# bd4sur/Nano

Measured on AMD Instinct MI355X. Metric: decode_tokens_per_sec, higher is better.
Workload: dtype i8

## Files before the change

nano_amd/csrc/gemv_q80_impl.h:

```cpp
#include <string.h>
#include <stdio.h>
#include "gemv_common.h"
#include "gemv_q80_host.h"

namespace nano {

namespace {


__device__ __forceinline__ void quant_store4(float4 v, float scale, int8_t *dst) {
    const int q0 = q80_quant1(v.x, scale), q1 = q80_quant1(v.y, scale), q2 = q80_quant1(v.z, scale), q3 = q80_quant1(v.w, scale);
    *reinterpret_cast<uint32_t *>(dst) = (uint32_t)(q0 & 0xff) | ((uint32_t)(q1 & 0xff) << 8) | ((uint32_t)(q2 & 0xff) << 16) | ((uint32_t)(q3 & 0xff) << 24);
}

template <int ROLE, int GS, int B, int NV>
__device__ __forceinline__ void stage_finish(const GemvDev &a, Staged<B, NV> &r, int8_t *xq, float *xs, float *red, uint32_t n16, uint32_t ng4) {
    const uint32_t tid = threadIdx.x, nthr = a.nthr, n = a.n, ng = a.ng;
    const uint32_t lane = tid & 63u, wid = tid >> 6, NW = nthr >> 6;
    if (has_flag<ROLE>(a, F_PRE)) {
        for (uint32_t b = 0; b < a.nb; b++) {
            for (uint32_t i = tid * 16u; i < n; i += nthr * 16u) *reinterpret_cast<int4 *>(xq + b * n16 + i) = *reinterpret_cast<const int4 *>(a.xq_in + (size_t)b * n16 + i);
            for (uint32_t i = tid; i < ng; i += nthr) xs[b * ng4 + i] = a.xs_in[(size_t)b * ng + i];
        }
        __syncthreads();
// ... 154 lines not shown
template <int NQ> __device__ __forceinline__ float fold_row_canon(const float *p) {
    static_assert(NQ % 2 == 0, "whole units");
    float4 t[NQ];
#pragma unroll
    for (int q = 0; q < NQ; q++) t[q] = *reinterpret_cast<const float4 *>(p + 4 * q);
    __builtin_amdgcn_sched_barrier(0);
    float s[NQ / 2];
    unit_sums<NQ / 2>(t, s);
    float v = s[0];
#pragma unroll
    for (int u = 1; u < NQ / 2; u++) v = fadd(v, s[u]);
    return v;
}
__device__ __forceinline__ float fold_row_canon_any(const float *p, uint32_t ng) {
    float v = 0.0f;
    for (uint32_t g0 = 0; g0 < ng; g0 += 16) {
        float4 t[4];
#pragma unroll
        for (int q = 0; q < 4; q++) t[q] = (g0 + 4u * (uint32_t)q < ng) ? *reinterpret_cast<const float4 *>(p + g0 + 4 * q) : make_float4(0.f, 0.f, 0.f, 0.f);
        float s = t[0].x; s += t[0].y; s += t[0].z; s += t[0].w;
        if (g0 + 4 < ng) { s += t[1].x; s += t[1].y; s += t[1].z; s += t[1].w; }
        v = g0 == 0 ? s : v + s;
        if (g0 + 8 < ng) {
            s = t[2].x; s += t[2].y; s += t[2].z; s += t[2].w;
            if (g0 + 12 < ng) { s += t[3].x; s += t[3].y; s += t[3].z; s += t[3].w; }
            v += s;
        }
    }
    return v;
}
template <int NQ> __device__ __forceinline__ void fold_row2_canon(const float *p0, const float *p1, float &v0, float &v1) {
    static_assert(NQ % 2 == 0, "whole units");
    float4 t[NQ], u[NQ];
#pragma unroll
    for (int q = 0; q < NQ; q++) { t[q] = *reinterpret_cast<const float4 *>(p0 + 4 * q); u[q] = *reinterpret_cast<const float4 *>(p1 + 4 * q); }
    __builtin_amdgcn_sched_barrier(0);
    float s0[NQ / 2], s1[NQ / 2];
    unit_sums<NQ / 2>(t, s0); unit_sums<NQ / 2>(u, s1);
    v0 = s0[0]; v1 = s1[0];
#pragma unroll
    for (int k = 1; k < NQ / 2; k++) { v0 = fadd(v0, s0[k]); v1 = fadd(v1, s1[k]); }
}
__device__ __forceinline__ void fold_row2_canon_ng(const float *p0, const float *p1, uint32_t ng, float &v0, float &v1) {
    if (ng == 16u) { fold_row2_canon<4>(p0, p1, v0, v1); return; }
    v0 = fold_row_canon_any(p0, ng); v1 = fold_row_canon_any(p1, ng);
}
__device__ __forceinline__ float fold_row_canon_ng(const float *p, uint32_t ng) {
    if (ng == 16u) return fold_row_canon<4>(p);
    if (ng == 32u) return fold_row_canon<8>(p);
    if (ng == 48u) return fold_row_canon<12>(p);
    return fold_row_canon_any(p, ng);
}

template <int ROLE, int GS, int B, int NV, int UPW, int EARLY = 0>
__global__ __launch_bounds__(1024) void gemv_q80_slab_kernel(const GemvDev a) {
    extern __shared__ __attribute__((aligned(16))) unsigned char smem[];
#define SLAB_EARLY EARLY
#define SLAB_A a
#define SLAB_BID blockIdx.x
#define SLAB_HAND 0
#define SLAB_HANDV (SlabHand{})
#define SLAB_PTAG 0u
#define SLAB_XHAND 0
#define SLAB_XHANDV (SlabHand{})
#define SLAB_CTAG 0u
#define SLAB_PART 0
#include "gemv_q80_slab_body.inc"
#undef SLAB_A
#undef SLAB_BID
#undef SLAB_HAND
#undef SLAB_HANDV
#undef SLAB_PTAG
#undef SLAB_XHAND
#undef SLAB_XHANDV
#undef SLAB_CTAG
#undef SLAB_PART
#undef SLAB_EARLY
}

#if NANO_Q80_GS == 64
}
}
#include "attn_impl.h"
namespace nano {
namespace {
struct FusedArgs { GemvDev g; AttnArgs a; SlabHand hand; uint32_t n_attn, head_wgs, wait16, ngemv; };
template <int NV, int UPW>
__global__ __launch_bounds__(256) void qkv_attn_fused_kernel(const FusedArgs fa) {
    extern __shared__ __attribute__((aligned(16))) unsigned char smem[];
    const uint2 tk_ = hand_tick(fa.hand);
    if (blockIdx.x >= fa.ngemv) {
        const uint32_t ab = blockIdx.x - fa.ngemv;
        const uint32_t split = ab / fa.head_wgs, grp = ab - split * fa.head_wgs;
        attention_body<8, 4, 1, 1, false, false, 2, false, true>(fa.a, smem, grp, 0u, split, fa.hand, hand_ctag(tk_, fa.hand), fa.wait16);
        return;
    }
    constexpr int ROLE = R_NORM_STORE, GS = 64, B = 1;
#define SLAB_A fa.g
#define SLAB_BID blockIdx.x
#define SLAB_HAND 1
#define SLAB_HANDV fa.hand
#define SLAB_PTAG hand_ptag(tk_, fa.hand)
#define SLAB_XHAND 0
#define SLAB_XHANDV (SlabHand{})
#define SLAB_CTAG 0u
#define SLAB_PART 0
#include "gemv_q80_slab_body.inc"
#undef SLAB_A
#undef SLAB_BID
#undef SLAB_HAND
#undef SLAB_HANDV
#undef SLAB_PTAG
#undef SLAB_XHAND
#undef SLAB_XHANDV
#undef SLAB_CTAG
#undef SLAB_PART
}

struct Wo13Args { GemvDev wo; GemvDev w13; SlabHand hand; uint32_t wo_wgs, wait16; };
template <int ROLE_A, int NV_A, int UPW_A, int NV_B, int UPW_B, int NT>
__global__ __launch_bounds__(NT) void wo_w13_fused_kernel(const Wo13Args fa) {
    extern __shared__ __attribute__((aligned(16))) unsigned char smem[];
    constexpr int GS = 64, B = 1;
    const uint2 tk_ = hand_tick(fa.hand);
    {
        constexpr int ROLE = ROLE_A, NV = NV_A, UPW = UPW_A;
#define SLAB_BID blockIdx.x
#define SLAB_A fa.wo
#define SLAB_HAND 1
#define SLAB_HANDV fa.hand
#define SLAB_PTAG hand_ptag(tk_, fa.hand)
#define SLAB_XHAND 0
#define SLAB_XHANDV (SlabHand{})
#define SLAB_CTAG 0u
#define SLAB_PART 1
#include "gemv_q80_slab_body.inc"
#undef SLAB_PART
        auto wo_rest = [&]() __attribute__((always_inline)) {
#define SLAB_PART 2
#include "gemv_q80_slab_body.inc"
#undef SLAB_PART
        };
#undef SLAB_A
#undef SLAB_HAND
#undef SLAB_HANDV
#undef SLAB_PTAG
#undef SLAB_XHAND
#undef SLAB_XHANDV
#undef SLAB_CTAG
        {
            constexpr int ROLE = R_NORM_SWIGLU, NV = NV_B, UPW = UPW_B;
#define SLAB_A fa.w13
#define SLAB_HAND 0
#define SLAB_HANDV (SlabHand{})
#define SLAB_PTAG 0u
#define SLAB_XHAND 1
#define SLAB_XHANDV fa.hand
#define SLAB_CTAG hand_ctag(tk_, fa.hand)
#define SLAB_XHAND_WAIT (blockIdx.x >= fa.wo_wgs ? fa.wait16 : 0u)
#define SLAB_XHAND_NAP 2
#define SLAB_PART 1
#include "gemv_q80_slab_body.inc"
#undef SLAB_PART
            if (blockIdx.x < fa.wo_wgs) wo_rest();
            __syncthreads();
#define SLAB_PART 2
#include "gemv_q80_slab_body.inc"
#undef SLAB_PART
#undef SLAB_A
#undef SLAB_HAND
#undef SLAB_HANDV
#undef SLAB_PTAG
#undef SLAB_XHAND
#undef SLAB_XHANDV
#undef SLAB_CTAG
#undef SLAB_XHAND_WAIT
#undef SLAB_XHAND_NAP
        }
#undef SLAB_BID
    }
}

#endif

template <int ROLE, int GS, int B, int NV>
__global__ __launch_bounds__(256) void gemv_q80_stream_kernel(const GemvDev a) {
    extern __shared__ __attribute__((aligned(16))) unsigned char smem[];
    constexpr int LPG = GS / 16, GC = 1024 / GS, F = GC / 4;
    static_assert(F >= 1, "group size too large for the stream kernel");
    const uint32_t n = a.n, ng = a.ng;
    const int tid = threadIdx.x, lane = tid & 63;
    const int wid = __builtin_amdgcn_readfirstlane(tid >> 6);
    const uint32_t n16 = (n + 15) & ~15u, ng4 = (ng + 3) & ~3u;
    int8_t *xq = reinterpret_cast<int8_t *>(smem);
    float *xs = reinterpret_cast<float *>(smem + B * n16);
    float *red = xs + B * ng4;
    int *tab = reinterpret_cast<int *>(red + B * 16) + wid * 16 * GC;

    Staged<B, NV> sx;
    stage_issue<ROLE, B, NV>(a, sx);

    const uint32_t rows = a.rows[0];
    const uint32_t nchunk = a.nchunk;
    const uint32_t ntiles = (rows + 15) >> 4;
    const uint32_t nwaves = gridDim.x * 4, wave_g = blockIdx.x * 4 + (uint32_t)wid;
    const uint32_t nunits = (wave_g < ntiles) ? ((ntiles - wave_g + nwaves - 1) / nwaves) * nchunk : 0;
    const __amdgpu_buffer_rsrc_t rw_ = mkrsrc(a.w[0], rows * n);
    const __amdgpu_buffer_rsrc_t rs_ = mkrsrc(a.ws[0], rows * ng * 4u);

    int4 wA[16];
    float sA[F];
    uint32_t tile_i = 0, chunk_i = 0;
    auto issue = [&](int4 (&w)[16], float (&s)[F]) {
        const uint32_t tile = wave_g + tile_i * nwaves;
        const uint32_t row0 = tile << 4;
        const uint32_t col = (chunk_i << 10) + (uint32_t)lane * 16u;
        const uint32_t base = (col < n) ? row0 * n + col : OOB;
#pragma unroll
        for (int r = 0; r < 16; r++) w[r] = bload_w(rw_, base + (uint32_t)r * n);
        const uint32_t gb = chunk_i * GC + ((uint32_t)lane & 3u) * F;
        const uint32_t so = ((row0 + ((uint32_t)lane >> 2)) * ng + gb) * 4u;
#pragma unroll
        for (int f = 0; f < F; f++) s[f] = bload_f(rs_, (gb + f < ng) ? so + 4u * f : OOB);
        if (++chunk_i == nchunk) { chunk_i = 0; tile_i++; }
    };
    if (nunits) issue(wA, sA);

    stage_finish<ROLE, GS, B, NV>(a, sx, xq, xs, red, n16, ng4);

    float val[B], best[B];
// ... 81 lines not shown
    const uint32_t nchunk = (a.n + 1023) / 1024, nmat = a.epi == GEMV_EPI_SWIGLU ? 2 : 1;
    const uint32_t nseg = a.epi == GEMV_EPI_SWIGLU ? 1u : a.nseg;
    uint32_t align = 0;
    if (nseg > 1) for (uint32_t s = 0; s < nseg; s++) align |= a.seg[s].rows;
    const uint32_t rows = total_rows(a);
    uint32_t rw = 4;
    while (rw < 32 && (align % (rw * 2)) == 0 && (rw * 2 / 4) * nchunk <= 4 && rows / (rw * 2) >= 128) rw *= 2;
    while (rw < 64 && (align % (rw * 2)) == 0 && rows / (rw * 2) >= 256) rw *= 2;
    {
        const uint32_t ng = a.n / a.gs, pitch = ((ng + 47) / 64) * 64 + 16;
        while (rw > 4 && (size_t)B * nmat * rw * pitch * 4 > 64 * 1024) rw /= 2;
        while (rw > 4 && (rw / 4) * nchunk * nmat > 64) rw /= 2;
    }
    if (B == 1 && nseg == 1) {
        const uint32_t cus = a.cus ? a.cus : 256u, c = (rows + cus - 1) / cus;
        if (c >= 5 && c < rw && rows / rw < cus && ((c + 3) / 4) * nchunk * nmat <= 64) rw = c;
    }
    uint32_t large_nw = 0;
    if (B <= 2 && (uint64_t)rows * a.n * nmat >= (8u << 20)) {
        const uint32_t cus = a.cus ? a.cus : 256u;
        uint32_t best = 0, best_cost = ~0u;
        const uint32_t ng = a.n / a.gs, pitch = (1024 / a.gs == 16) ? (((ng + 47) / 64) * 64 + 16) : (((ng + 3) & ~3u) + 4);
        for (uint32_t c = 4; c <= 64; c++) {
            const uint32_t tpw = (c + 3) / 4;
            if (tpw * nchunk * nmat > 64) break;
            if ((size_t)B * nmat * tpw * 4 * pitch * 4 > 96 * 1024) break;
            uint32_t wgs = 0;
            if (nseg > 1) for (uint32_t s2 = 0; s2 < nseg; s2++) wgs += (a.seg[s2].rows + c - 1) / c; else wgs = (rows + c - 1) / c;
            uint32_t cost = ((wgs + cus - 1) / cus) * c * 100u;
            if (wgs > cus) cost += cost * 15u / 100u;
            if (cost <= best_cost) { best_cost = cost; best = c; }
        }
        if (best) {
            rw = best;
            const uint32_t u = ((rw + 3) / 4) * nchunk * nmat;
            large_nw = u / 2 < 8 ? 8 : (u / 2 > 16 ? 16 : u / 2);
        }
    }
    const uint32_t units = ((rw + 3) / 4) * nchunk * nmat;
    uint32_t nw = units < 4 ? units : 4;
    const uint32_t want_div = B == 1 ? 384u : 512u;
    uint32_t want = (a.n * (uint32_t)(B > 2 ? B / 2 : 1) + want_div - 1) / want_div;
    if (want > 16) want = 16;
    if (nw < want) nw = want;
    if (nw * 64 < rw * (uint32_t)B) nw = (rw * (uint32_t)B + 63) / 64;
    if (nw < 2) nw = 2;
    uint32_t upw = (units + nw - 1) / nw;
    while (upw > 4 && nw < 16) { nw++; upw = (units + nw - 1) / nw; }
    if (large_nw) { nw = large_nw; upw = (units + nw - 1) / nw; while (upw > 4 && nw < 16) { nw++; upw = (units + nw - 1) / nw; } }
    SlabPlan p{rw, nw, upw, (a.n + 256 * nw - 1) / (256 * nw)};
    return p;
}

template <int ROLE, int GS, int B, int NV, int UPW>
static hipError_t launch_slab_t(const GemvDev &d, const SlabPlan &p, uint32_t nwg, hipStream_t st) {
    const uint32_t nmat = d.epi == GEMV_EPI_SWIGLU ? 2 : 1;
    const size_t n16 = (d.n + 15) & ~15u, ng4 = (d.ng + 3) & ~3u;
    const size_t pitch = (1024 / GS == 16) ? (((d.ng + 47) / 64) * 64 + 16) : (ng4 + 4);
    const size_t lds = B * n16 + B * ng4 * 4 + B * 64 + ((d.flags & F_COMBINE) ? (size_t)B * d.attn_n_head * 32 : 0) + (size_t)B * nmat * (d.tpw * 4) * pitch * 4;
    GemvDev dd = d; dd.nthr = 64 * p.nw;
    if constexpr (GS == 64 && B <= 2 && UPW >= 2 && NV >= 1) if (d.early) {
        auto kern = &gemv_q80_slab_kernel<ROLE, GS, B, NV, UPW, 1>;
        if (lds > 64 * 1024) (void)hipFuncSetAttribute(reinterpret_cast<const void *>(kern), hipFuncAttributeMaxDynamicSharedMemorySize, (int)lds);
        hipLaunchKernelGGL(kern, dim3(nwg), dim3(64 * p.nw), lds, st, dd);
        return hipGetLastError();
    }
    auto kern = &gemv_q80_slab_kernel<ROLE, GS, B, NV, UPW>;
    if (lds > 64 * 1024) (void)hipFuncSetAttribute(reinterpret_cast<const void *>(kern), hipFuncAttributeMaxDynamicSharedMemorySize, (int)lds);
    hipLaunchKernelGGL(kern, dim3(nwg), dim3(64 * p.nw), lds, st, dd);
    return hipGetLastError();
}
template <int ROLE, int GS, int B>
static hipError_t launch_slab_r(const GemvDev &d, const SlabPlan &p, uint32_t rows, hipStream_t st) {
    if (p.upw > 4) return hipErrorInvalidValue;
#define SLAB_GO(NV_, UPW_) do { if constexpr (B * NV_ <= 8) return launch_slab_t<ROLE, GS, B, NV_, UPW_>(d, p, rows, st); } while (0)
    int nv = p.nv <= 1 ? 1 : p.nv <= 2 ? 2 : p.nv <= 4 ? 4 : 0;
    const int upw = p.upw <= 1 ? 1 : p.upw <= 2 ? 2 : 4;
    if (B * nv > 8) nv = 0;
    if (nv == 1) { if (upw == 1) SLAB_GO(1, 1); if (upw == 2) SLAB_GO(1, 2); SLAB_GO(1, 4); }
    if (nv == 2) { if (upw == 1) SLAB_GO(2, 1); if (upw == 2) SLAB_GO(2, 2); SLAB_GO(2, 4); }
    if (nv == 4) { if (upw == 1) SLAB_GO(4, 1); if (upw == 2) SLAB_GO(4, 2); SLAB_GO(4, 4); }
    if (upw == 1) SLAB_GO(0, 1);
    if (upw == 2) SLAB_GO(0, 2);
    SLAB_GO(0, 4);
    return hipErrorInvalidValue;
#undef SLAB_GO
}
template <int GS, int B>
static hipError_t launch_slab_b(GemvDev &d, const GemvArgs &a, hipStream_t st) {
    const SlabPlan p = plan_slab(a, B);
    d.rw = p.rw;
    d.early = (B <= 2 && p.upw >= 2 && (uint64_t)total_rows(a) * a.n * (a.epi == GEMV_EPI_SWIGLU ? 2 : 1) >= (8u << 20)) ? 1u : 0u;
    d.tpw = (p.rw + 3) / 4;
    d.magic_rw = 65536u / p.rw + 1u;
    d.log2_tiles = 0;
    const bool sw = d.epi == GEMV_EPI_SWIGLU;
    d.units = d.tpw * d.nchunk * (sw ? 2 : 1);
    uint32_t wg[3] = {0, 0, 0};
    const uint32_t nseg = sw ? 1u : a.nseg;
    for (uint32_t s2 = 0; s2 < nseg; s2++) wg[s2] = (a.seg[s2].rows + p.rw - 1) / p.rw;
    d.wg_c0 = nseg > 1 ? wg[0] : 0xffffffffu;
    d.wg_c1 = nseg > 2 ? wg[0] + wg[1] : 0xffffffffu;
    const uint32_t rows = wg[0] + wg[1] + wg[2];
    if constexpr (B == 1) if (GS != 64 || d.canon) {
        const uint32_t f = d.flags;
        if (f == F_NORM && d.epi == GEMV_EPI_STORE) return launch_slab_r<R_NORM_STORE, GS, B>(d, p, rows, st);
        if (f == 0 && d.epi == GEMV_EPI_RESID) return launch_slab_r<R_RESID, GS, B>(d, p, rows, st);
        if (f == F_COMBINE && d.epi == GEMV_EPI_RESID) return launch_slab_r<R_RESID_COMBINE, GS, B>(d, p, rows, st);
        if (f == F_NORM && d.epi == GEMV_EPI_SWIGLU) return launch_slab_r<R_NORM_SWIGLU, GS, B>(d, p, rows, st);
    }
    return launch_slab_r<R_GENERIC, GS, B>(d, p, rows, st);
}

template <int ROLE, int GS, int B>
static hipError_t launch_stream_r(GemvDev &d, hipStream_t st) {
    d.ntiles = STREAM_WGS * 4; d.nthr = 256;
    const size_t n16 = (d.n + 15) & ~15u, ng4 = (d.ng + 3) & ~3u;
// ... 9 lines not shown
    if constexpr (B <= 2) { if (!done && nv <= 4) { STREAM_GO(4); done = true; } }
    if (!done) { STREAM_GO(0); }
#undef STREAM_GO
    return hipGetLastError();
}
template <int GS, int B>
static hipError_t launch_stream_b(GemvDev &d, hipStream_t st) {
    if (d.flags == F_NORM) return launch_stream_r<R_NORM_STORE, GS, B>(d, st);
    return launch_stream_r<R_GENERIC, GS, B>(d, st);
}

#if NANO_Q80_GS == 64
static bool fused_shape(const GemvArgs &ga, const AttnArgs &aa, SlabPlan &p) {
    if (ga.gs != 64 || ga.nb != 1 || ga.nseg != 3 || ga.epi != GEMV_EPI_STORE || !ga.norm_w || ga.xq_in || ga.attn_part || ga.tile_max || ga.resid_add) return false;
    if (ga.n % 64u || ga.n > 4096u || use_stream(ga) || !q80_canonical(ga)) return false;
    if (ga.seg[0].out_pstride || ga.seg[1].out_pstride) return false;
    p = plan_slab(ga, 1);
    if (p.nw != 4u || p.upw > 4u || !(p.nv == 1u || p.nv == 2u || p.nv == 4u)) return false;
    if (!fused_attn_side_ok(aa, ga.seg[0].rows, ga.seg[1].rows, ga.seg[2].rows)) return false;
    return true;
}

struct Wo13Plan { SlabPlan a, b; uint32_t nw, nv_a, upw_a, wa, wb; int sig; };
static bool wo13_shape(const GemvArgs &wo, const GemvArgs &w13, Wo13Plan &q) {
    if (wo.gs != 64 || w13.gs != 64 || wo.nb != 1 || w13.nb != 1 || !q80_canonical(wo) || !q80_canonical(w13)) return false;
    if (wo.nseg != 1 || wo.epi != GEMV_EPI_RESID || wo.norm_w || wo.xq_in || wo.tile_max || wo.resid_add || wo.seg[0].out_pstride) return false;
    if (wo.attn_part && (wo.attn_nsplit > 8u || wo.attn_hd % 4u)) return false;
    if (w13.nseg != 2 || w13.epi != GEMV_EPI_SWIGLU || !w13.norm_w || w13.xq_in || w13.attn_part || w13.tile_max || w13.resid_add) return false;
    if (use_stream(wo) || use_stream(w13) || w13.n != wo.seg[0].rows || w13.xin != wo.seg[0].out || w13.n % 4u) return false;
    q.a = plan_slab(wo, 1); q.b = plan_slab(w13, 1);
    q.nw = q.b.nw;
    const uint32_t units_a = ((q.a.rw + 3) / 4) * ((wo.n + 1023) / 1024);
    q.upw_a = (units_a + q.nw - 1) / q.nw;
    q.nv_a = (wo.n / 4 + 64 * q.nw - 1) / (64 * q.nw);
    q.wa = (wo.seg[0].rows + q.a.rw - 1) / q.a.rw; q.wb = (w13.seg[0].rows + q.b.rw - 1) / q.b.rw;
    const uint32_t cus = w13.cus ? w13.cus : 256u;
    if (q.wa > q.wb || q.wb > cus) return false;
    if (q.a.rw > 64 * q.nw || q.b.rw > 64 * q.nw) return false;
    q.sig = 0;
    if (q.nw == 4u && q.nv_a == 2u && q.upw_a == 1u && q.b.nv == 1u && q.b.upw == 2u) q.sig = 1;
    if (q.sig == 1) {
        const uint32_t units_b = ((q.b.rw + 3) / 4) * ((w13.n + 1023) / 1024) * 2u;
        if ((units_a + 7u) / 8u == 1u && (wo.n / 4 + 511u) / 512u == 1u && (units_b + 7u) / 8u == 1u && (w13.n / 4 + 511u) / 512u == 1u) { q.sig = 3; q.nw = 8u; }
    }
    return q.sig != 0;
}
static void slab_dev_fill(GemvDev &d, const GemvArgs &a, const SlabPlan &p, uint32_t nthr) {
    d.tile_max = nullptr;
    d.rw = p.rw; d.tpw = (p.rw + 3) / 4; d.magic_rw = 65536u / p.rw + 1u; d.log2_tiles = 0;
    d.units = d.tpw * d.nchunk * (a.epi == GEMV_EPI_SWIGLU ? 2u : 1u);
    d.wg_c0 = 0xffffffffu; d.wg_c1 = 0xffffffffu;
    d.nthr = nthr;
}
static size_t slab_lds(const GemvDev &d) {
    const uint32_t nmat = d.epi == GEMV_EPI_SWIGLU ? 2 : 1;
    const size_t n16 = (d.n + 15) & ~15u, ng4 = (d.ng + 3) & ~3u, pitch = ((d.ng + 47) / 64) * 64 + 16;
    return n16 + ng4 * 4 + 64 + ((d.flags & F_COMBINE) ? (size_t)d.attn_n_head * 32 : 0) + (size_t)nmat * (d.tpw * 4) * pitch * 4;
}

#endif

template <int GS, int B>
static hipError_t launch_b(const GemvArgs &a, hipStream_t st) {
    GemvDev d = to_dev(a);
    if (use_stream(a)) return launch_stream_b<GS, B>(d, st);
    d.tile_max = nullptr;
    return launch_slab_b<GS, B>(d, a, st);
}
template <int GS>
static hipError_t launch_gs(const GemvArgs &a, hipStream_t st) {
    if (a.nb <= 1) return launch_b<GS, 1>(a, st);
    if (a.nb <= 2) return launch_b<GS, 2>(a, st);
    if (a.nb <= 4) return launch_b<GS, 4>(a, st);
    return launch_b<GS, 8>(a, st);
}

}

hipError_t NANO_Q80_ENTRY(const GemvArgs &a, hipStream_t st) { return launch_gs<NANO_Q80_GS>(a, st); }

#if NANO_Q80_GS == 64
bool qkv_attn_fused_supports(const GemvArgs &ga, const AttnArgs &aa) { SlabPlan p; return fused_shape(ga, aa, p); }

hipError_t launch_qkv_attn_fused(const GemvArgs &ga, const AttnArgs &aa, unsigned long long *hand, uint32_t *tick, uint32_t layer1, hipStream_t st) {
    SlabPlan p;
    if (!hand || !tick || !layer1 || layer1 > 127u || !fused_shape(ga, aa, p)) return hipErrorInvalidValue;
    GemvDev d = to_dev(ga);
    d.tile_max = nullptr;
    d.rw = p.rw; d.tpw = (p.rw + 3) / 4; d.magic_rw = 65536u / p.rw + 1u; d.log2_tiles = 0;
    d.units = d.tpw * d.nchunk;
    uint32_t wg[3];
    for (uint32_t s2 = 0; s2 < 3; s2++) wg[s2] = (ga.seg[s2].rows + p.rw - 1) / p.rw;
    d.wg_c0 = wg[0]; d.wg_c1 = wg[0] + wg[1];
    const uint32_t ngemv = wg[0] + wg[1] + wg[2];
    d.nthr = 256;
    AttnArgs a = aa;
    { uint32_t l2 = 0; while ((1u << l2) < a.n_kv_head) l2++; a.kv_log2 = l2; }
    { const uint32_t kv_mul = a.n_head / a.n_kv_head; uint32_t l2 = 0; while ((1u << l2) < kv_mul) l2++; a.kvmul_log2 = l2; }
    SlabHand h{};
    h.buf = hand; h.tick = tick; h.layer1 = layer1;
    h.base[0] = 0; h.base[1] = a.q_dim; h.base[2] = a.q_dim + a.kv_dim;
    const uint32_t n_attn = a.n_head * a.nsplit;
    const size_t n16 = (d.n + 15) & ~15u, ng4 = (d.ng + 3) & ~3u, pitch = ((d.ng + 47) / 64) * 64 + 16;
    const size_t lds_g = n16 + ng4 * 4 + 64 + (size_t)(d.tpw * 4) * pitch * 4;
    const size_t hd4 = a.hd, lds_a = (hd4 + hd4 + 4 + 4 + 4 * hd4 + hd4 + 4 + 4 * 8 * hd4) * sizeof(float);
    const size_t lds = lds_g > lds_a ? lds_g : lds_a;
    if (lds > 64 * 1024) return hipErrorInvalidValue;
    const int upw = p.upw <= 1 ? 1 : p.upw <= 2 ? 2 : 4;
    FusedArgs fa{};
    fa.g = d; fa.a = a; fa.hand = h; fa.n_attn = n_attn; fa.head_wgs = a.n_head; fa.ngemv = ngemv;
    fa.wait16 = 1u;
#define FUSED_GO(NV_, UPW_) do { hipLaunchKernelGGL((qkv_attn_fused_kernel<NV_, UPW_>), dim3(n_attn + ngemv), dim3(256), lds, st, fa); return hipGetLastError(); } while (0)
#define FUSED_NV(NV_) do { if (upw == 1) FUSED_GO(NV_, 1); if (upw == 2) FUSED_GO(NV_, 2); FUSED_GO(NV_, 4); } while (0)
    if (p.nv == 1u) FUSED_NV(1);
    if (p.nv == 2u) FUSED_NV(2);
    FUSED_NV(4);
#undef FUSED_NV
#undef FUSED_GO
}

bool wo_w13_fused_supports(const GemvArgs &wo, const GemvArgs &w13) { Wo13Plan q; return wo13_shape(wo, w13, q); }

hipError_t launch_wo_w13_fused(const GemvArgs &wo, const GemvArgs &w13, unsigned long long *hand, uint32_t *tick, uint32_t layer1, hipStream_t st) {
    Wo13Plan q;
    if (!hand || !tick || !layer1 || layer1 > 127u || !wo13_shape(wo, w13, q)) return hipErrorInvalidValue;
    Wo13Args fa{};
    fa.wo = to_dev(wo); fa.w13 = to_dev(w13);
    slab_dev_fill(fa.wo, wo, q.a, 64 * q.nw); slab_dev_fill(fa.w13, w13, q.b, 64 * q.nw);
    fa.wo_wgs = q.wa;
    fa.wait16 = 4u;
    SlabHand h{};
    h.buf = hand; h.tick = tick; h.layer1 = layer1;
    h.base[0] = 0; h.base[1] = 0; h.base[2] = 0;
    fa.hand = h;
    const size_t la = slab_lds(fa.wo), lb = slab_lds(fa.w13), lds = la > lb ? la : lb;
    if (lds > 64 * 1024) return hipErrorInvalidValue;
    const bool comb = (fa.wo.flags & F_COMBINE) != 0;
#define WO13_GO(RA_, NVA_, UA_, NVB_, UB_, NT_) do { hipLaunchKernelGGL((wo_w13_fused_kernel<RA_, NVA_, UA_, NVB_, UB_, NT_>), dim3(q.wb), dim3(NT_), lds, st, fa); return hipGetLastError(); } while (0)
    if (q.sig == 1) { if (comb) WO13_GO(R_RESID_COMBINE, 2, 1, 1, 2, 256); WO13_GO(R_RESID, 2, 1, 1, 2, 256); }
    if (comb) WO13_GO(R_RESID_COMBINE, 1, 1, 1, 1, 512);
    WO13_GO(R_RESID, 1, 1, 1, 1, 512);
#undef WO13_GO
}
#endif

}
```

nano_amd/csrc/gemv_q80_slab_body.inc:

```
#ifndef SLAB_EARLY
#define SLAB_EARLY 0
#define SLAB_EARLY_DEFAULTED 1
#endif
#ifndef SLAB_XHAND_WAIT
#define SLAB_XHAND_WAIT 0u
#define SLAB_XHAND_NAP 0
#define SLAB_XHAND_WAIT_DEFAULTED 1
#endif
#define SLAB_ISSUE_UNIT(k) do { \
        const uint32_t u = (uint32_t)wid + (uint32_t)k * NW; \
        const uint32_t t = (u * SLAB_A.magic_nchunk) >> 16; \
        const uint32_t c = u - t * SLAB_A.nchunk; \
        const uint32_t mat = t >= TPW ? 1u : 0u, tl = t - mat * TPW; \
        const bool live = u < SLAB_A.units; \
        const __amdgpu_buffer_rsrc_t rw_ = mkrsrc(mat ? SLAB_A.w[1] : w0, live ? rows0 * n : 0u); \
        const __amdgpu_buffer_rsrc_t rs_ = mkrsrc(mat ? SLAB_A.ws[1] : ws0, live ? rows0 * ng * 4u : 0u); \
        const uint32_t lrow = lrow0 + tl * TR; \
        const uint32_t col = (c << 10) + (uint32_t)lane * 16u; \
        const uint32_t base = (col < n) ? lrow * n + col : OOB; \
        _Pragma("unroll") \
        for (int r = 0; r < TR; r++) wv[k][r] = bload_w(rw_, base + ((tl * TR + (uint32_t)r < RW) ? (uint32_t)r * n : OOB)); \
        const uint32_t g = c * GC + (uint32_t)lane / LPG; \
        _Pragma("unroll") \
        for (int s = 0; s < NS; s++) { \
            const uint32_t r = ((uint32_t)lane % LPG) + s * LPG; \
            sv[k][s] = bload_f(rs_, (r < TR && tl * TR + r < RW && g < ng) ? ((lrow + r) * ng + g) * 4u : OOB); \
        } \
    } while (0)
#if SLAB_PART != 2
    constexpr int TR = 4;
    constexpr int LPG = GS / 16, GC = 1024 / GS;
    constexpr int NS = (TR + LPG - 1) / LPG;
    const int tid = threadIdx.x, lane = tid & 63;
    const int wid = __builtin_amdgcn_readfirstlane(tid >> 6);
    const int NW = (int)(SLAB_A.nthr >> 6);
    const uint32_t n = SLAB_A.n, ng = SLAB_A.ng;
    const uint32_t n16 = (n + 15) & ~15u, ng4 = (ng + 3) & ~3u;
    const uint32_t PITCH = (GC == 16) ? (((ng + 47) / 64) * 64 + 16) : (ng4 + 4);
    const uint32_t RW = SLAB_A.rw, TPW = SLAB_A.tpw, RWP = TPW * TR;
    const uint32_t epi = role_epi<ROLE>(SLAB_A);
    const bool swiglu = epi == GEMV_EPI_SWIGLU;
    const uint32_t nmat = swiglu ? 2 : 1;
    int8_t *xq = reinterpret_cast<int8_t *>(smem);
    float *xs = reinterpret_cast<float *>(smem + B * n16);
    float *red = xs + B * ng4;
    float *P = red + B * 16 + (has_flag<ROLE>(SLAB_A, F_COMBINE) ? B * SLAB_A.attn_n_head * 8 : 0);

    karg_touch(SLAB_A.out[0]); karg_touch(SLAB_A.out_bstride[0]); karg_touch(SLAB_A.out_pstride[0]); karg_touch(SLAB_A.rows[0]); karg_touch(SLAB_A.magic_rw); karg_touch(SLAB_A.nb);
    if (!(ROLE == R_RESID || ROLE == R_RESID_COMBINE || ROLE == R_NORM_SWIGLU)) {
        karg_touch(SLAB_A.out[1]); karg_touch(SLAB_A.out[2]); karg_touch(SLAB_A.out_bstride[1]); karg_touch(SLAB_A.out_bstride[2]);
        karg_touch(SLAB_A.out_pstride[1]); karg_touch(SLAB_A.out_pstride[2]); karg_touch(SLAB_A.rows[1]); karg_touch(SLAB_A.rows[2]);
    }
    karg_touch(SLAB_A.pos); karg_touch(SLAB_A.canon);
    if (ROLE == R_GENERIC || ROLE == R_RESID || ROLE == R_RESID_COMBINE) { karg_touch(SLAB_A.resid_add); karg_touch(SLAB_A.resid_add_bstride); }
    NANO_STAMP(SLAB_A.stamps, 0, tid);
    Staged<B, NV> sx;
    if constexpr (SLAB_XHAND) stage_issue_nw<ROLE, B, NV>(SLAB_A, sx);
    else if (!(NANO_STAMPS && (SLAB_A.dbg & 2u))) stage_issue<ROLE, B, NV>(SLAB_A, sx);

    constexpr bool ONESEG = ROLE == R_RESID || ROLE == R_RESID_COMBINE || ROLE == R_NORM_SWIGLU;
    const int sel = (ONESEG || swiglu) ? 0 : (int)(SLAB_BID >= SLAB_A.wg_c0) + (int)(SLAB_BID >= SLAB_A.wg_c1);
    const int8_t *w0 = sel == 0 ? SLAB_A.w[0] : sel == 1 ? SLAB_A.w[1] : SLAB_A.w[2];
    const float *ws0 = sel == 0 ? SLAB_A.ws[0] : sel == 1 ? SLAB_A.ws[1] : SLAB_A.ws[2];
    float *out0 = sel == 0 ? SLAB_A.out[0] : sel == 1 ? SLAB_A.out[1] : SLAB_A.out[2];
    const uint32_t rows0 = sel == 0 ? SLAB_A.rows[0] : sel == 1 ? SLAB_A.rows[1] : SLAB_A.rows[2];
    const uint32_t obs = sel == 0 ? SLAB_A.out_bstride[0] : sel == 1 ? SLAB_A.out_bstride[1] : SLAB_A.out_bstride[2];
    const uint32_t ops = sel == 0 ? SLAB_A.out_pstride[0] : sel == 1 ? SLAB_A.out_pstride[1] : SLAB_A.out_pstride[2];
    const uint32_t lrow0 = (SLAB_BID - (sel == 0 ? 0u : sel == 1 ? SLAB_A.wg_c0 : SLAB_A.wg_c1)) * RW;

    int4 wv[UPW][TR];
    float sv[UPW][NS];
    constexpr uint32_t early_ = (uint32_t)(SLAB_EARLY);
    static_assert(SLAB_PART == 0 || early_ == 0u, "SLAB_EARLY: the whole body only");
#pragma unroll
    for (int k = 0; k < UPW; k++) { if (early_ == 0u || (uint32_t)k < early_) SLAB_ISSUE_UNIT(k); }
    if (!SLAB_XHAND && NANO_STAMPS && (SLAB_A.dbg & 2u)) stage_issue<ROLE, B, NV>(SLAB_A, sx);
    const int fb = (int)(((uint32_t)tid * SLAB_A.magic_rw) >> 16);
    const int frl = tid - fb * (int)RW;
    const bool fold_live = tid < (int)(RW * B) && fb < (int)SLAB_A.nb && lrow0 + frl < rows0;
    uint32_t opos = 0;
    if (ops && fold_live) opos = SLAB_A.pos[fb];
    float oldv = 0.0f;
    if (epi == GEMV_EPI_RESID && fold_live) oldv = out0[(size_t)fb * obs + lrow0 + frl];
    float addv = 0.0f;
    const bool has_add = epi == GEMV_EPI_RESID && SLAB_A.resid_add != nullptr;
    if (has_add && fold_live) addv = SLAB_A.resid_add[(size_t)fb * SLAB_A.resid_add_bstride + lrow0 + frl];

    NANO_STAMP(SLAB_A.stamps, 1, oldv);
#endif
#if SLAB_PART != 1
    if constexpr (SLAB_XHAND) {
        static_assert(!SLAB_XHAND || B == 1, "granule activations: one sequence");
        const unsigned long long *hb_ = SLAB_XHANDV.buf;
        const uint32_t ctag_ = SLAB_CTAG;
        bool got_ = false;
        for (uint32_t w_ = 0; w_ < SLAB_XHAND_WAIT; w_++) __builtin_amdgcn_s_sleep(16);
        for (uint32_t spin_ = 0; spin_ < (1u << 14) && !got_; spin_++) {
            if (spin_) __builtin_amdgcn_s_sleep(SLAB_XHAND_NAP);
            if ((spin_ & 63u) == 63u && hand_aborted(SLAB_XHANDV)) break;
            got_ = true;
#pragma unroll
            for (int j = 0; j < NV; j++) {
                const uint32_t i = ((uint32_t)tid + (uint32_t)j * SLAB_A.nthr) * 4u;
                if (i < n) {
                    const unsigned long long g0_ = __hip_atomic_load(hb_ + i, __ATOMIC_RELAXED, __HIP_MEMORY_SCOPE_AGENT);
                    const unsigned long long g1_ = __hip_atomic_load(hb_ + i + 1, __ATOMIC_RELAXED, __HIP_MEMORY_SCOPE_AGENT);
                    const unsigned long long g2_ = __hip_atomic_load(hb_ + i + 2, __ATOMIC_RELAXED, __HIP_MEMORY_SCOPE_AGENT);
                    const unsigned long long g3_ = __hip_atomic_load(hb_ + i + 3, __ATOMIC_RELAXED, __HIP_MEMORY_SCOPE_AGENT);
                    got_ = got_ && (uint32_t)(g0_ >> 32) == ctag_ && (uint32_t)(g1_ >> 32) == ctag_ && (uint32_t)(g2_ >> 32) == ctag_ && (uint32_t)(g3_ >> 32) == ctag_;
                    sx.x[0][j] = make_float4(__uint_as_float((uint32_t)g0_), __uint_as_float((uint32_t)g1_), __uint_as_float((uint32_t)g2_), __uint_as_float((uint32_t)g3_));
                } else sx.x[0][j] = make_float4(0.f, 0.f, 0.f, 0.f);
            }
        }
        if (!got_) hand_give_up(SLAB_XHANDV, SLAB_A.err);
    }
    stage_finish<ROLE, GS, B, NV>(SLAB_A, sx, xq, xs, red, n16, ng4);
    if constexpr (early_ != 0u) {
#pragma unroll
        for (int k = 1; k < UPW; k++) { if ((uint32_t)k >= early_) SLAB_ISSUE_UNIT(k); }
    }
    NANO_STAMP(SLAB_A.stamps, 3, xs[0]);

#pragma unroll
    for (int k = 0; k < UPW; k++) {
        const uint32_t u = (uint32_t)wid + (uint32_t)k * NW;
        if (u < SLAB_A.units) {
            const uint32_t t = (u * SLAB_A.magic_nchunk) >> 16;
            const uint32_t c = u - t * SLAB_A.nchunk;
            const uint32_t mat = t >= TPW ? 1u : 0u, tl = t - mat * TPW;
            const uint32_t col = (c << 10) + (uint32_t)lane * 16u;
            const uint32_t g = c * GC + (uint32_t)lane / LPG;
#pragma unroll
            for (int b = 0; b < B; b++) {
                if (b < (int)SLAB_A.nb) {
                    const int4 xv = (col < n) ? *reinterpret_cast<const int4 *>(xq + b * n16 + col) : make_int4(0, 0, 0, 0);
                    int iv[TR];
#pragma unroll
                    for (int r = 0; r < TR; r++) {
                        int d = __builtin_amdgcn_sdot4(wv[k][r].x, xv.x, 0, false);
                        d = __builtin_amdgcn_sdot4(wv[k][r].y, xv.y, d, false);
                        d = __builtin_amdgcn_sdot4(wv[k][r].z, xv.z, d, false);
                        d = __builtin_amdgcn_sdot4(wv[k][r].w, xv.w, d, false);
                        iv[r] = dpp_group_sum<LPG>(d);
                    }
                    const float xsc = (g < ng) ? xs[b * ng4 + g] : 0.0f;
#pragma unroll
                    for (int s = 0; s < NS; s++) {
                        const uint32_t r = ((uint32_t)lane % LPG) + s * LPG;
                        int v = iv[0];
#pragma unroll
                        for (int q = 1; q < TR; q++) v = (q == (int)r) ? iv[q] : v;
                        if (r < TR && g < ng)
                            P[(((size_t)b * nmat + mat) * RWP + tl * TR + r) * PITCH + g] = ((float)v * sv[k][s]) * xsc;
                    }
                }
            }
        }
    }
    NANO_STAMP(SLAB_A.stamps, 4, wv[UPW - 1][TR - 1].w);
    __syncthreads();
    NANO_STAMP(SLAB_A.stamps, 5, P[0]);

    constexpr bool PFOLD = early_ != 0u && GS == 64;
    bool pfold_ = false;
    if constexpr (PFOLD) {
        pfold_ = (ROLE != R_GENERIC || SLAB_A.canon) && (ng & 7u) == 0u;
        if (pfold_) {
            const uint32_t nu_ = ng >> 3, rows_ = RW * (uint32_t)B * nmat, items_ = rows_ * nu_;
            for (uint32_t it = (uint32_t)tid; it < items_; it += SLAB_A.nthr) {
                const uint32_t rr_ = it / nu_, u_ = it - rr_ * nu_;
                const uint32_t bm_ = rr_ / RW, rl_ = rr_ - bm_ * RW;
                float *pu_ = P + ((size_t)bm_ * RWP + rl_) * PITCH + 8u * u_;
                const float4 t0_ = *reinterpret_cast<const float4 *>(pu_), t1_ = *reinterpret_cast<const float4 *>(pu_ + 4);
                pu_[0] = unit_sum(t0_, t1_);
            }
// ... 15 lines not shown
            if constexpr (ROLE == R_NORM_SWIGLU) fold_row2_canon_ng(p0, p1, ng, v0, v1); else v0 = fold_row_canon_ng(p0, ng);
        } else
        if (GS == 64 && SLAB_A.canon) {
            v0 = fold_row_canon_ng(p0, ng);
            if (swiglu) v1 = fold_row_canon_ng(p1, ng);
        } else
        if (!swiglu && ng == 48u) v0 = fold_row<12>(p0);
        else if (!swiglu && ng == 32u) v0 = fold_row<8>(p0);
        else if (ng == 16u) {
            if (swiglu) fold_row2<4>(p0, p1, v0, v1); else v0 = fold_row<4>(p0);
        } else if ((ng & 15u) == 0) {
            for (uint32_t g0 = 0; g0 < ng; g0 += 16) {
                float4 t[4], u[4];
#pragma unroll
                for (int q = 0; q < 4; q++) { t[q] = *reinterpret_cast<const float4 *>(p0 + g0 + 4 * q); if (swiglu) u[q] = *reinterpret_cast<const float4 *>(p1 + g0 + 4 * q); }
#pragma unroll
                for (int q = 0; q < 4; q++) { v0 += t[q].x; v0 += t[q].y; v0 += t[q].z; v0 += t[q].w; }
                if (swiglu) {
#pragma unroll
                    for (int q = 0; q < 4; q++) { v1 += u[q].x; v1 += u[q].y; v1 += u[q].z; v1 += u[q].w; }
                }
            }
        } else {
        for (uint32_t g0 = 0; g0 < ng; g0 += 16) {
                float4 t[4], u[4];
#pragma unroll
                for (int q = 0; q < 4; q++) {
                    t[q] = (g0 + 4 * q < ng4) ? *reinterpret_cast<const float4 *>(p0 + g0 + 4 * q) : make_float4(0.f, 0.f, 0.f, 0.f);
                    if (swiglu) u[q] = (g0 + 4 * q < ng4) ? *reinterpret_cast<const float4 *>(p1 + g0 + 4 * q) : make_float4(0.f, 0.f, 0.f, 0.f);
                }
#pragma unroll
                for (int q = 0; q < 4; q++) {
                    const uint32_t g = g0 + 4 * q;
                    v0 += (g < ng) ? t[q].x : 0.0f; v0 += (g + 1 < ng) ? t[q].y : 0.0f; v0 += (g + 2 < ng) ? t[q].z : 0.0f; v0 += (g + 3 < ng) ? t[q].w : 0.0f;
                }
                if (swiglu) {
#pragma unroll
                    for (int q = 0; q < 4; q++) {
                        const uint32_t g = g0 + 4 * q;
                        v1 += (g < ng) ? u[q].x : 0.0f; v1 += (g + 1 < ng) ? u[q].y : 0.0f; v1 += (g + 2 < ng) ? u[q].z : 0.0f; v1 += (g + 3 < ng) ? u[q].w : 0.0f;
                    }
                }
            }
        }
        if (fold_live) {
            float *dst = out0 + (size_t)fb * obs + (size_t)opos * ops + lrow0 + frl;
            const float val = finish_epi(epi, has_add ? v0 + addv : v0, v1, oldv);
            if constexpr (SLAB_HAND == 1)
                __hip_atomic_store(SLAB_HANDV.buf + (sel == 0 ? SLAB_HANDV.base[0] : sel == 1 ? SLAB_HANDV.base[1] : SLAB_HANDV.base[2]) + lrow0 + (uint32_t)frl,
                                   ((unsigned long long)(SLAB_PTAG) << 32) | (unsigned long long)__float_as_uint(val), __ATOMIC_RELAXED, __HIP_MEMORY_SCOPE_AGENT);
            if (NANO_STAMPS && (SLAB_A.dbg & 4u)) *dst = val; else __hip_atomic_store(dst, val, __ATOMIC_RELAXED, __HIP_MEMORY_SCOPE_AGENT);
        }
    }
    NANO_STAMP_END(SLAB_A.stamps, 6);
#endif
#undef SLAB_ISSUE_UNIT
#ifdef SLAB_EARLY_DEFAULTED
#undef SLAB_EARLY
#undef SLAB_EARLY_DEFAULTED
#endif
#ifdef SLAB_XHAND_WAIT_DEFAULTED
#undef SLAB_XHAND_WAIT
#undef SLAB_XHAND_NAP
#undef SLAB_XHAND_WAIT_DEFAULTED
#endif
```

Measured before the change: 1969.

## Add wave-level cross-lane fold path for single-chunk rmsnorm GEMVs

Adds a specialised slab-kernel variant for n=1024, 16-group rmsnorm-store and swiglu GEMVs. Each wave reduces its rows entirely in registers using DPP and permlane16/32 swaps, instead of writing partial sums to an LDS table and folding them after a barrier. The swiglu variant pairs the gate and up rows within one unit, which halves the unit count, and the LDS partial table is dropped from the allocation. This removes LDS traffic and synchronisation in the small-model decode GEMVs, at the cost of extra template instantiations and a hardcoded shape path.

```diff
diff --git a/nano_amd/csrc/gemv_q80_impl.h b/nano_amd/csrc/gemv_q80_impl.h
--- a/nano_amd/csrc/gemv_q80_impl.h
+++ b/nano_amd/csrc/gemv_q80_impl.h
@@ -230,10 +230,23 @@
     return fold_row_canon_any(p, ng);
 }
 
-template <int ROLE, int GS, int B, int NV, int UPW, int EARLY = 0>
+__device__ __forceinline__ float wave_fold_canon16(float p) {
+    const float p1 = DPP_F(p, 0x104), p2 = DPP_F(p, 0x108), p3 = DPP_F(p, 0x10C);
+    float s = fadd(p, p1); s = fadd(s, p2); s = fadd(s, p3);
+    const uint32_t sb = __float_as_uint(s);
+    const float c = __uint_as_float(__builtin_amdgcn_permlane16_swap(sb, sb, false, false)[0]);
+    s = fadd(c, p); s = fadd(s, p1); s = fadd(s, p2); s = fadd(s, p3);
+    const uint32_t tb = __float_as_uint(s);
+    const float s0 = __uint_as_float(__builtin_amdgcn_permlane32_swap(tb, tb, false, false)[0]);
+    return fadd(s0, s);
+}
+constexpr int WF_LANE0 = 48;
+
+template <int ROLE, int GS, int B, int NV, int UPW, int EARLY = 0, int WF = 0>
 __global__ __launch_bounds__(1024) void gemv_q80_slab_kernel(const GemvDev a) {
     extern __shared__ __attribute__((aligned(16))) unsigned char smem[];
 #define SLAB_EARLY EARLY
+#define SLAB_WF WF
 #define SLAB_A a
 #define SLAB_BID blockIdx.x
 #define SLAB_HAND 0
@@ -254,6 +267,7 @@
 #undef SLAB_CTAG
 #undef SLAB_PART
 #undef SLAB_EARLY
+#undef SLAB_WF
 }
 
 #if NANO_Q80_GS == 64
@@ -265,38 +279,19 @@
 struct FusedArgs { GemvDev g; AttnArgs a; SlabHand hand; uint32_t n_attn, head_wgs, wait16, ngemv; };
 template <int NV, int UPW>
 __global__ __launch_bounds__(256) void qkv_attn_fused_kernel(const FusedArgs fa) {
-    extern __shared__ __attribute__((aligned(16))) unsigned char smem[];
-    const uint2 tk_ = hand_tick(fa.hand);
-    if (blockIdx.x >= fa.ngemv) {
-        const uint32_t ab = blockIdx.x - fa.ngemv;
-        const uint32_t split = ab / fa.head_wgs, grp = ab - split * fa.head_wgs;
-        attention_body<8, 4, 1, 1, false, false, 2, false, true>(fa.a, smem, grp, 0u, split, fa.hand, hand_ctag(tk_, fa.hand), fa.wait16);
-        return;
-    }
-    constexpr int ROLE = R_NORM_STORE, GS = 64, B = 1;
-#define SLAB_A fa.g
-#define SLAB_BID blockIdx.x
-#define SLAB_HAND 1
-#define SLAB_HANDV fa.hand
-#define SLAB_PTAG hand_ptag(tk_, fa.hand)
-#define SLAB_XHAND 0
-#define SLAB_XHANDV (SlabHand{})
-#define SLAB_CTAG 0u
-#define SLAB_PART 0
-#include "gemv_q80_slab_body.inc"
-#undef SLAB_A
-#undef SLAB_BID
-#undef SLAB_HAND
-#undef SLAB_HANDV
-#undef SLAB_PTAG
-#undef SLAB_XHAND
-#undef SLAB_XHANDV
-#undef SLAB_CTAG
-#undef SLAB_PART
+#define SLAB_WF 0
+#include "qkv_attn_fused_body.inc"
+#undef SLAB_WF
+}
+template <int NV, int UPW>
+__global__ __launch_bounds__(256) void qkv_attn_fused_wf_kernel(const FusedArgs fa) {
+#define SLAB_WF 1
+#include "qkv_attn_fused_body.inc"
+#undef SLAB_WF
 }
 
 struct Wo13Args { GemvDev wo; GemvDev w13; SlabHand hand; uint32_t wo_wgs, wait16; };
-template <int ROLE_A, int NV_A, int UPW_A, int NV_B, int UPW_B, int NT>
+template <int ROLE_A, int NV_A, int UPW_A, int NV_B, int UPW_B, int NT, int WF = 0>
 __global__ __launch_bounds__(NT) void wo_w13_fused_kernel(const Wo13Args fa) {
     extern __shared__ __attribute__((aligned(16))) unsigned char smem[];
     constexpr int GS = 64, B = 1;
@@ -337,6 +332,7 @@
 #define SLAB_CTAG hand_ctag(tk_, fa.hand)
 #define SLAB_XHAND_WAIT (blockIdx.x >= fa.wo_wgs ? fa.wait16 : 0u)
 #define SLAB_XHAND_NAP 2
+#define SLAB_WF WF
 #define SLAB_PART 1
 #include "gemv_q80_slab_body.inc"
 #undef SLAB_PART
@@ -354,6 +350,7 @@
 #undef SLAB_CTAG
 #undef SLAB_XHAND_WAIT
 #undef SLAB_XHAND_NAP
+#undef SLAB_WF
         }
 #undef SLAB_BID
     }
@@ -541,6 +538,9 @@
     return p;
 }
 
+static bool slab_wave_fold(const GemvDev &d) {
+    return d.n == 1024u && d.ng == 16u && !d.early && (d.epi == GEMV_EPI_STORE || (d.epi == GEMV_EPI_SWIGLU && !d.out_pstride[0]));
+}
 template <int ROLE, int GS, int B, int NV, int UPW>
 static hipError_t launch_slab_t(const GemvDev &d, const SlabPlan &p, uint32_t nwg, hipStream_t st) {
     const uint32_t nmat = d.epi == GEMV_EPI_SWIGLU ? 2 : 1;
@@ -552,6 +552,11 @@
         auto kern = &gemv_q80_slab_kernel<ROLE, GS, B, NV, UPW, 1>;
         if (lds > 64 * 1024) (void)hipFuncSetAttribute(reinterpret_cast<const void *>(kern), hipFuncAttributeMaxDynamicSharedMemorySize, (int)lds);
         hipLaunchKernelGGL(kern, dim3(nwg), dim3(64 * p.nw), lds, st, dd);
+        return hipGetLastError();
+    }
+    if constexpr (GS == 64 && B == 1 && (ROLE == R_NORM_STORE || ROLE == R_NORM_SWIGLU) && (NV == 1 || NV == 2)) if (slab_wave_fold(d)) {
+        if (ROLE == R_NORM_SWIGLU) dd.units = (d.rw + 1) / 2;
+        hipLaunchKernelGGL((gemv_q80_slab_kernel<ROLE, GS, B, NV, UPW, 0, 1>), dim3(nwg), dim3(64 * p.nw), n16 + ng4 * 4 + 64, st, dd);
         return hipGetLastError();
     }
     auto kern = &gemv_q80_slab_kernel<ROLE, GS, B, NV, UPW>;
@@ -667,10 +672,10 @@
     d.wg_c0 = 0xffffffffu; d.wg_c1 = 0xffffffffu;
     d.nthr = nthr;
 }
-static size_t slab_lds(const GemvDev &d) {
+static size_t slab_lds(const GemvDev &d, bool table = true) {
     const uint32_t nmat = d.epi == GEMV_EPI_SWIGLU ? 2 : 1;
     const size_t n16 = (d.n + 15) & ~15u, ng4 = (d.ng + 3) & ~3u, pitch = ((d.ng + 47) / 64) * 64 + 16;
-    return n16 + ng4 * 4 + 64 + ((d.flags & F_COMBINE) ? (size_t)d.attn_n_head * 32 : 0) + (size_t)nmat * (d.tpw * 4) * pitch * 4;
+    return n16 + ng4 * 4 + 64 + ((d.flags & F_COMBINE) ? (size_t)d.attn_n_head * 32 : 0) + (table ? (size_t)nmat * (d.tpw * 4) * pitch * 4 : 0);
 }
 
 #endif
@@ -717,7 +722,8 @@
     h.base[0] = 0; h.base[1] = a.q_dim; h.base[2] = a.q_dim + a.kv_dim;
     const uint32_t n_attn = a.n_head * a.nsplit;
     const size_t n16 = (d.n + 15) & ~15u, ng4 = (d.ng + 3) & ~3u, pitch = ((d.ng + 47) / 64) * 64 + 16;
-    const size_t lds_g = n16 + ng4 * 4 + 64 + (size_t)(d.tpw * 4) * pitch * 4;
+    const bool wf = slab_wave_fold(d);
+    const size_t lds_g = n16 + ng4 * 4 + 64 + (wf ? 0 : (size_t)(d.tpw * 4) * pitch * 4);
     const size_t hd4 = a.hd, lds_a = (hd4 + hd4 + 4 + 4 + 4 * hd4 + hd4 + 4 + 4 * 8 * hd4) * sizeof(float);
     const size_t lds = lds_g > lds_a ? lds_g : lds_a;
     if (lds > 64 * 1024) return hipErrorInvalidValue;
@@ -725,7 +731,8 @@
     FusedArgs fa{};
     fa.g = d; fa.a = a; fa.hand = h; fa.n_attn = n_attn; fa.head_wgs = a.n_head; fa.ngemv = ngemv;
     fa.wait16 = 1u;
-#define FUSED_GO(NV_, UPW_) do { hipLaunchKernelGGL((qkv_attn_fused_kernel<NV_, UPW_>), dim3(n_attn + ngemv), dim3(256), lds, st, fa); return hipGetLastError(); } while (0)
+#define FUSED_GO(NV_, UPW_) do { if (wf && NV_ == 1) hipLaunchKernelGGL((qkv_attn_fused_wf_kernel<1, UPW_>), dim3(n_attn + ngemv), dim3(256), lds, st, fa); \
+                                 else hipLaunchKernelGGL((qkv_attn_fused_kernel<NV_, UPW_>), dim3(n_attn + ngemv), dim3(256), lds, st, fa); return hipGetLastError(); } while (0)
 #define FUSED_NV(NV_) do { if (upw == 1) FUSED_GO(NV_, 1); if (upw == 2) FUSED_GO(NV_, 2); FUSED_GO(NV_, 4); } while (0)
     if (p.nv == 1u) FUSED_NV(1);
     if (p.nv == 2u) FUSED_NV(2);
@@ -748,10 +755,13 @@
     h.buf = hand; h.tick = tick; h.layer1 = layer1;
     h.base[0] = 0; h.base[1] = 0; h.base[2] = 0;
     fa.hand = h;
-    const size_t la = slab_lds(fa.wo), lb = slab_lds(fa.w13), lds = la > lb ? la : lb;
+    const bool wf = slab_wave_fold(fa.w13);
+    if (wf) fa.w13.units = (fa.w13.rw + 1) / 2;
+    const size_t la = slab_lds(fa.wo), lb = slab_lds(fa.w13, !wf), lds = la > lb ? la : lb;
     if (lds > 64 * 1024) return hipErrorInvalidValue;
     const bool comb = (fa.wo.flags & F_COMBINE) != 0;
-#define WO13_GO(RA_, NVA_, UA_, NVB_, UB_, NT_) do { hipLaunchKernelGGL((wo_w13_fused_kernel<RA_, NVA_, UA_, NVB_, UB_, NT_>), dim3(q.wb), dim3(NT_), lds, st, fa); return hipGetLastError(); } while (0)
+#define WO13_GO(RA_, NVA_, UA_, NVB_, UB_, NT_) do { if (wf) hipLaunchKernelGGL((wo_w13_fused_kernel<RA_, NVA_, UA_, NVB_, UB_, NT_, 1>), dim3(q.wb), dim3(NT_), lds, st, fa); \
+                                                     else hipLaunchKernelGGL((wo_w13_fused_kernel<RA_, NVA_, UA_, NVB_, UB_, NT_>), dim3(q.wb), dim3(NT_), lds, st, fa); return hipGetLastError(); } while (0)
     if (q.sig == 1) { if (comb) WO13_GO(R_RESID_COMBINE, 2, 1, 1, 2, 256); WO13_GO(R_RESID, 2, 1, 1, 2, 256); }
     if (comb) WO13_GO(R_RESID_COMBINE, 1, 1, 1, 1, 512);
     WO13_GO(R_RESID, 1, 1, 1, 1, 512);
diff --git a/nano_amd/csrc/gemv_q80_slab_body.inc b/nano_amd/csrc/gemv_q80_slab_body.inc
--- a/nano_amd/csrc/gemv_q80_slab_body.inc
+++ b/nano_amd/csrc/gemv_q80_slab_body.inc
@@ -1,3 +1,7 @@
+#ifndef SLAB_WF
+#define SLAB_WF 0
+#define SLAB_WF_DEFAULTED 1
+#endif
 #ifndef SLAB_EARLY
 #define SLAB_EARLY 0
 #define SLAB_EARLY_DEFAULTED 1
@@ -8,6 +12,21 @@
 #define SLAB_XHAND_WAIT_DEFAULTED 1
 #endif
 #define SLAB_ISSUE_UNIT(k) do { \
+      if constexpr (WFPAIR_) { \
+         \
+         \
+        const uint32_t u = (uint32_t)wid + (uint32_t)k * NW; \
+        const bool live = u < SLAB_A.units; \
+        const __amdgpu_buffer_rsrc_t rw0_ = mkrsrc(w0, live ? rows0 * n : 0u), rw1_ = mkrsrc(SLAB_A.w[1], live ? rows0 * n : 0u); \
+        const __amdgpu_buffer_rsrc_t rs0_ = mkrsrc(ws0, live ? rows0 * ng * 4u : 0u), rs1_ = mkrsrc(SLAB_A.ws[1], live ? rows0 * ng * 4u : 0u); \
+        const uint32_t lrow = lrow0 + u * 2u, base = lrow * n + (uint32_t)lane * 16u; \
+        _Pragma("unroll") \
+        for (int r = 0; r < TR; r++) wv[k][r] = bload_w(r < 2 ? rw0_ : rw1_, (u * 2u + (uint32_t)(r & 1) < RW) ? base + (uint32_t)(r & 1) * n : OOB); \
+        const uint32_t r_ = (uint32_t)lane & 3u, rr_ = r_ & 1u; \
+        const uint32_t so_ = (u * 2u + rr_ < RW) ? ((lrow + rr_) * ng + ((uint32_t)lane >> 2)) * 4u : OOB; \
+        const float s0_ = bload_f(rs0_, r_ < 2u ? so_ : OOB), s1_ = bload_f(rs1_, r_ < 2u ? OOB : so_); \
+        sv[k][0] = __uint_as_float(__float_as_uint(s0_) | __float_as_uint(s1_)); \
+      } else { \
         const uint32_t u = (uint32_t)wid + (uint32_t)k * NW; \
         const uint32_t t = (u * SLAB_A.magic_nchunk) >> 16; \
         const uint32_t c = u - t * SLAB_A.nchunk; \
@@ -26,6 +45,7 @@
             const uint32_t r = ((uint32_t)lane % LPG) + s * LPG; \
             sv[k][s] = bload_f(rs_, (r < TR && tl * TR + r < RW && g < ng) ? ((lrow + r) * ng + g) * 4u : OOB); \
         } \
+      } \
     } while (0)
 #if SLAB_PART != 2
     constexpr int TR = 4;
@@ -34,7 +54,9 @@
     const int tid = threadIdx.x, lane = tid & 63;
     const int wid = __builtin_amdgcn_readfirstlane(tid >> 6);
     const int NW = (int)(SLAB_A.nthr >> 6);
-    const uint32_t n = SLAB_A.n, ng = SLAB_A.ng;
+    constexpr bool WF_ = (SLAB_WF) != 0, WFPAIR_ = WF_ && ROLE == R_NORM_SWIGLU;
+    static_assert(!WF_ || (GS == 64 && B == 1 && (SLAB_EARLY) == 0 && (ROLE == R_NORM_STORE || ROLE == R_NORM_SWIGLU)), "SLAB_WF: one-chunk rows of the rmsnorm roles");
+    const uint32_t n = WF_ ? 1024u : SLAB_A.n, ng = WF_ ? 16u : SLAB_A.ng;
     const uint32_t n16 = (n + 15) & ~15u, ng4 = (ng + 3) & ~3u;
     const uint32_t PITCH = (GC == 16) ? (((ng + 47) / 64) * 64 + 16) : (ng4 + 4);
     const uint32_t RW = SLAB_A.rw, TPW = SLAB_A.tpw, RWP = TPW * TR;
@@ -79,6 +101,9 @@
     const int frl = tid - fb * (int)RW;
     const bool fold_live = tid < (int)(RW * B) && fb < (int)SLAB_A.nb && lrow0 + frl < rows0;
     uint32_t opos = 0;
+    if constexpr (WF_) {
+        if constexpr (ROLE == R_NORM_STORE) opos = __float_as_uint(bload_f(mkrsrc(SLAB_A.pos, ops ? 4u : 0u), ((uint32_t)lane & ~3u) == (uint32_t)WF_LANE0 ? 0u : OOB));
+    } else
     if (ops && fold_live) opos = SLAB_A.pos[fb];
     float oldv = 0.0f;
     if (epi == GEMV_EPI_RESID && fold_live) oldv = out0[(size_t)fb * obs + lrow0 + frl];
@@ -121,6 +146,48 @@
     }
     NANO_STAMP(SLAB_A.stamps, 3, xs[0]);
 
+    if constexpr (WF_) {
+    float pw_[UPW];
+    const int4 xv_ = *reinterpret_cast<const int4 *>(xq + lane * 16);
+    const float xsc_ = xs[lane >> 2];
+    asm volatile("" :: "v"(xsc_));
+#pragma unroll
+    for (int k = 0; k < UPW; k++) {
+        int iv[TR];
+#pragma unroll
+        for (int r = 0; r < TR; r++) {
+            int d = __builtin_amdgcn_sdot4(wv[k][r].x, xv_.x, 0, false);
+            d = __builtin_amdgcn_sdot4(wv[k][r].y, xv_.y, d, false);
+            d = __builtin_amdgcn_sdot4(wv[k][r].z, xv_.z, d, false);
+            d = __builtin_amdgcn_sdot4(wv[k][r].w, xv_.w, d, false);
+            iv[r] = dpp_group_sum<LPG>(d);
+        }
+        int v = iv[0];
+#pragma unroll
+        for (int q = 1; q < TR; q++) v = (q == (lane & 3)) ? iv[q] : v;
+        pw_[k] = ((float)v * sv[k][0]) * xsc_;
+    }
+    NANO_STAMP(SLAB_A.stamps, 4, pw_[UPW - 1]);
+    NANO_STAMP(SLAB_A.stamps, 5, pw_[UPW - 1]);
+#pragma unroll
+    for (int k = 0; k < UPW; k++) {
+        const uint32_t u = (uint32_t)wid + (uint32_t)k * NW;
+        if (u < SLAB_A.units) {
+            const float v0 = wave_fold_canon16(pw_[k]);
+            const float v1 = WFPAIR_ ? DPP_F(v0, 0x102) : 0.0f;
+            const uint32_t rl_ = WFPAIR_ ? u * 2u + ((uint32_t)lane & 1u) : u * (uint32_t)TR + ((uint32_t)lane & 3u);
+            const bool mine_ = WFPAIR_ ? ((uint32_t)lane & ~1u) == (uint32_t)WF_LANE0 : ((uint32_t)lane & ~3u) == (uint32_t)WF_LANE0;
+            if (mine_ && rl_ < RW && lrow0 + rl_ < rows0) {
+                float *dst = out0 + (size_t)opos * ops + lrow0 + rl_;
+                const float val = finish_epi(epi, v0, v1, 0.0f);
+                if constexpr (SLAB_HAND == 1)
+                    __hip_atomic_store(SLAB_HANDV.buf + (sel == 0 ? SLAB_HANDV.base[0] : sel == 1 ? SLAB_HANDV.base[1] : SLAB_HANDV.base[2]) + lrow0 + rl_,
+                                       ((unsigned long long)(SLAB_PTAG) << 32) | (unsigned long long)__float_as_uint(val), __ATOMIC_RELAXED, __HIP_MEMORY_SCOPE_AGENT);
+                if (NANO_STAMPS && (SLAB_A.dbg & 4u)) *dst = val; else __hip_atomic_store(dst, val, __ATOMIC_RELAXED, __HIP_MEMORY_SCOPE_AGENT);
+            }
+        }
+    }
+    } else {
 #pragma unroll
     for (int k = 0; k < UPW; k++) {
         const uint32_t u = (uint32_t)wid + (uint32_t)k * NW;
@@ -242,9 +309,14 @@
             if (NANO_STAMPS && (SLAB_A.dbg & 4u)) *dst = val; else __hip_atomic_store(dst, val, __ATOMIC_RELAXED, __HIP_MEMORY_SCOPE_AGENT);
         }
     }
+    }
     NANO_STAMP_END(SLAB_A.stamps, 6);
 #endif
 #undef SLAB_ISSUE_UNIT
+#ifdef SLAB_WF_DEFAULTED
+#undef SLAB_WF
+#undef SLAB_WF_DEFAULTED
+#endif
 #ifdef SLAB_EARLY_DEFAULTED
 #undef SLAB_EARLY
 #undef SLAB_EARLY_DEFAULTED
diff --git a/nano_amd/csrc/qkv_attn_fused_body.inc b/nano_amd/csrc/qkv_attn_fused_body.inc
--- /dev/null
+++ b/nano_amd/csrc/qkv_attn_fused_body.inc
@@ -0,0 +1,28 @@
+    extern __shared__ __attribute__((aligned(16))) unsigned char smem[];
+    const uint2 tk_ = hand_tick(fa.hand);
+    if (blockIdx.x >= fa.ngemv) {
+        const uint32_t ab = blockIdx.x - fa.ngemv;
+        const uint32_t split = ab / fa.head_wgs, grp = ab - split * fa.head_wgs;
+        attention_body<8, 4, 1, 1, false, false, 2, false, true>(fa.a, smem, grp, 0u, split, fa.hand, hand_ctag(tk_, fa.hand), fa.wait16);
+        return;
+    }
+    constexpr int ROLE = R_NORM_STORE, GS = 64, B = 1;
+#define SLAB_A fa.g
+#define SLAB_BID blockIdx.x
+#define SLAB_HAND 1
+#define SLAB_HANDV fa.hand
+#define SLAB_PTAG hand_ptag(tk_, fa.hand)
+#define SLAB_XHAND 0
+#define SLAB_XHANDV (SlabHand{})
+#define SLAB_CTAG 0u
+#define SLAB_PART 0
+#include "gemv_q80_slab_body.inc"
+#undef SLAB_A
+#undef SLAB_BID
+#undef SLAB_HAND
+#undef SLAB_HANDV
+#undef SLAB_PTAG
+#undef SLAB_XHAND
+#undef SLAB_XHANDV
+#undef SLAB_CTAG
+#undef SLAB_PART
```

After: 1994 (median of 6 runs). 1.01x the previous value.
